# qutech/filter_functions

Measured on AMD Instinct MI355X. Metric: filter-function elements/sec (n_seg*n_omega*n_nops*d^2) at d=4, higher is better.
Workload: dtype f64

## Files before the change

filter_functions_amd/csrc/post.hip:

```cpp
#include <algorithm>

#include <cstdlib>

#include "ffk_internal.h"

namespace ffk {
namespace {

__global__ void reduce_chunks_kernel(const cplx* __restrict__ Ypart, int chunks, size_t slab,
                                     cplx* __restrict__ Bt) {
    const size_t e = static_cast<size_t>(blockIdx.x)*blockDim.x + threadIdx.x;
    if (e >= slab) return;
    cplx acc = Ypart[e];
    for (int c = 1; c < chunks; ++c) {
        const cplx v = Ypart[static_cast<size_t>(c)*slab + e];
        acc.re += v.re;
        acc.im += v.im;
    }
    Bt[e] = acc;
}

__global__ __launch_bounds__(64) void basis_compact_kernel(const cplx* __restrict__ basis, int d,
                                                           int* __restrict__ nnz,
                                                           int* __restrict__ rows,
                                                           cplx* __restrict__ vals) {
    basis_compact_one(basis, d, blockIdx.x, threadIdx.x, nnz, rows, vals);
}

__global__ __launch_bounds__(256) void reduce_compact_kernel(const cplx* __restrict__ Ypart,
                                                             int chunks, size_t slab,
                                                             cplx* __restrict__ Bt, int nred,
                                                             const cplx* __restrict__ basis, int d,
                                                             int* __restrict__ nnz,
                                                             int* __restrict__ rows,
                                                             cplx* __restrict__ vals) {
    if (static_cast<int>(blockIdx.x) >= nred) {
        if (threadIdx.x < 64)
            basis_compact_one(basis, d, static_cast<int>(blockIdx.x) - nred, threadIdx.x, nnz, rows, vals);
        return;
    }
    const size_t e = static_cast<size_t>(blockIdx.x)*blockDim.x + threadIdx.x;
    if (e >= slab) return;
    cplx acc = Ypart[e];
    for (int c = 1; c < chunks; ++c) {
        const cplx v = Ypart[static_cast<size_t>(c)*slab + e];
        acc.re += v.re;
        acc.im += v.im;
    }
    Bt[e] = acc;
}

__device__ __forceinline__ bool basis_is_sparse(const int* __restrict__ nnz, int N, int dd) {
    int part = 0;
    for (int k = threadIdx.x & 63; k < N; k += 64) part += nnz[k];
#pragma unroll
    for (int off = 32; off > 0; off >>= 1) part += __shfl_xor(part, off, 64);
    return part <= 3*dd;
}

template <int KT>
__global__ __launch_bounds__(64) void expand_sparse_kernel(const cplx* __restrict__ Bt,
                                                           const int* __restrict__ nnz,
                                                           const int* __restrict__ rows,
                                                           const cplx* __restrict__ vals, int N,
                                                           int dd, int W, cplx* __restrict__ R,
                                                           int want_sparse) {
    if (want_sparse >= 0 && basis_is_sparse(nnz, N, dd) != (want_sparse != 0)) return;
    const int w = blockIdx.x*64 + threadIdx.x;
    const int a = blockIdx.y;
    if (w >= W) return;
    const cplx* b = Bt + static_cast<size_t>(a)*dd*W + w;
    for (int kk = 0; kk < KT; ++kk) {
        const int k = blockIdx.z*KT + kk;
        if (k >= N) break;
        const int n = nnz[k];
        const int* rk = rows + static_cast<size_t>(k)*dd;
        const cplx* vk = vals + static_cast<size_t>(k)*dd;
        cplx acc0 = {0.0, 0.0}, acc1 = {0.0, 0.0};
        int q = 0;
        for (; q + 1 < n; q += 2) {
            cmac(acc0, vk[q], b[static_cast<size_t>(rk[q])*W]);
            cmac(acc1, vk[q + 1], b[static_cast<size_t>(rk[q + 1])*W]);
        }
        if (q < n) cmac(acc0, vk[q], b[static_cast<size_t>(rk[q])*W]);
        R[(static_cast<size_t>(a)*N + k)*W + w] = {acc0.re + acc1.re, acc0.im + acc1.im};
    }
}
// ... 442 lines not shown

}

hipError_t launch_reduce_chunks(const cplx* Ypart, int chunks, size_t slab, cplx* Bt,
                                hipStream_t stream) {
    const int block = 256;
    hipLaunchKernelGGL(reduce_chunks_kernel, dim3(static_cast<unsigned>((slab + block - 1)/block)),
                       dim3(block), 0, stream, Ypart, chunks, slab, Bt);
    return hipGetLastError();
}

size_t expand_workspace_bytes(int N, int d) {
    const size_t dd = static_cast<size_t>(d)*d;
    return align_up(sizeof(int)*N) + align_up(sizeof(int)*N*dd) + align_up(sizeof(cplx)*N*dd);
}

namespace {
struct CompactWs {
    int* nnz;
    int* rows;
    cplx* vals;
};
CompactWs slice_compact_ws(void* ws, int N, int d) {
    const size_t dd = static_cast<size_t>(d)*d;
    unsigned char* p = static_cast<unsigned char*>(ws);
    CompactWs out;
    out.nnz = reinterpret_cast<int*>(p);
    p += align_up(sizeof(int)*N);
    out.rows = reinterpret_cast<int*>(p);
    p += align_up(sizeof(int)*N*dd);
    out.vals = reinterpret_cast<cplx*>(p);
    return out;
}
}

hipError_t launch_reduce_and_compact(const cplx* Ypart, int chunks, size_t slab, cplx* Bt,
                                     const cplx* basis, int N, int d, void* ws, hipStream_t stream) {
    const CompactWs c = slice_compact_ws(ws, N, d);
    const int block = 256;
    const int nred = static_cast<int>((slab + block - 1)/block);
    hipLaunchKernelGGL(reduce_compact_kernel, dim3(nred + N), dim3(block), 0, stream, Ypart, chunks,
                       slab, Bt, nred, basis, d, c.nnz, c.rows, c.vals);
    return hipGetLastError();
}

void expand_workspace_slices(void* ws, int N, int d, int** nnz, int** rows, cplx** vals) {
    const CompactWs cw = slice_compact_ws(ws, N, d);
    *nnz = cw.nnz;
    *rows = cw.rows;
    *vals = cw.vals;
}

__global__ __launch_bounds__(64) void expand_chunks_kernel(const cplx* __restrict__ Ypart, int chunks,
                                                           size_t slab, const int* __restrict__ nnz,
                                                           const int* __restrict__ rows,
                                                           const cplx* __restrict__ vals, int N,
                                                           int dd, int W, cplx* __restrict__ R) {
    const int w = blockIdx.x*64 + threadIdx.x;
    const int a = blockIdx.y, k = blockIdx.z;
    if (w >= W) return;
    const cplx* b = Ypart + static_cast<size_t>(a)*dd*W + w;
    const int n = nnz[k];
    const int* rk = rows + static_cast<size_t>(k)*dd;
    const cplx* vk = vals + static_cast<size_t>(k)*dd;
    auto summed = [&](int e) {
        cplx acc = b[static_cast<size_t>(e)*W];
        for (int z = 1; z < chunks; ++z) {
            const cplx v = b[z*slab + static_cast<size_t>(e)*W];
            acc.re += v.re;
            acc.im += v.im;
        }
        return acc;
    };
    cplx acc0 = {0.0, 0.0}, acc1 = {0.0, 0.0};
    int q = 0;
    for (; q + 1 < n; q += 2) {
        cmac(acc0, vk[q], summed(rk[q]));
        cmac(acc1, vk[q + 1], summed(rk[q + 1]));
    }
    if (q < n) cmac(acc0, vk[q], summed(rk[q]));
    R[(static_cast<size_t>(a)*N + k)*W + w] = {acc0.re + acc1.re, acc0.im + acc1.im};
}

__device__ __forceinline__ void expand_ff_tile(const cplx* __restrict__ Ypart, int chunks, size_t slab,
                                               const int* __restrict__ nnz, const int* __restrict__ rows,
                                               const cplx* __restrict__ vals, int N, int dd, int W, int A,
                                               int kt, cplx* __restrict__ R, cplx* __restrict__ F) {
    extern __shared__ __attribute__((aligned(16))) unsigned char lds_raw[];
    cplx* rl = reinterpret_cast<cplx*>(lds_raw);
    __builtin_amdgcn_s_setprio(3);
    cplx* ys = rl + static_cast<size_t>(A)*N*16;
    const int wl = threadIdx.x & 15;
    const int kl = (threadIdx.x >> 4) % kt, al = (threadIdx.x >> 4) / kt;
    const int at = (blockDim.x >> 4) / kt;
    const int w = blockIdx.x*16 + wl;
    const int wc = w < W ? w : W - 1;
    for (int idx = threadIdx.x >> 4; idx < A*dd; idx += blockDim.x >> 4) {
        const cplx* b = Ypart + static_cast<size_t>(idx)*W + wc;
        cplx acc = b[0];
        for (int z = 1; z < chunks; ++z) {
            const cplx v = b[z*slab];
            acc.re += v.re;
            acc.im += v.im;
        }
        ys[static_cast<size_t>(idx)*16 + wl] = acc;
    }
    __syncthreads();
    for (int a = al; a < A; a += at) {
        const cplx* ya = ys + static_cast<size_t>(a)*dd*16 + wl;
        for (int k = kl; k < N; k += kt) {
            const int n = nnz[k];
            const int* rk = rows + static_cast<size_t>(k)*dd;
            const cplx* vk = vals + static_cast<size_t>(k)*dd;
            auto summed = [&](int e) { return ya[e*16]; };
            cplx acc0 = {0.0, 0.0}, acc1 = {0.0, 0.0};
            int q = 0;
            for (; q + 1 < n; q += 2) {
                cmac(acc0, vk[q], summed(rk[q]));
                cmac(acc1, vk[q + 1], summed(rk[q + 1]));
            }
            if (q < n) cmac(acc0, vk[q], summed(rk[q]));
            const cplx r = {acc0.re + acc1.re, acc0.im + acc1.im};
            rl[(static_cast<size_t>(a)*N + k)*16 + wl] = r;
            if (w < W) R[(static_cast<size_t>(a)*N + k)*W + w] = r;
        }
    }
    __syncthreads();
    if (w >= W) return;
    const int npairs = A*(A + 1)/2;
    const int lanes = blockDim.x >> 4;
    for (int p = threadIdx.x >> 4; p < npairs; p += lanes) {
        int a = 0, rem = p;
        while (rem >= A - a) {
            rem -= A - a;
            ++a;
        }
        const int b = a + rem;
        const cplx* ra = rl + static_cast<size_t>(a)*N*16 + wl;
        const cplx* rb = rl + static_cast<size_t>(b)*N*16 + wl;
        cplx acc = {0.0, 0.0};
        for (int k = 0; k < N; ++k) cmac_conj(acc, ra[k*16], rb[k*16]);
        if (a == b) acc.im = 0.0;
        F[(static_cast<size_t>(a)*A + b)*W + w] = acc;
        if (a != b) F[(static_cast<size_t>(b)*A + a)*W + w] = {acc.re, -acc.im};
    }
}

__global__ __launch_bounds__(256) void expand_ff_kernel(const cplx* __restrict__ Ypart, int chunks,
                                                         size_t slab, const int* __restrict__ nnz,
                                                         const int* __restrict__ rows,
                                                         const cplx* __restrict__ vals, int N, int dd,
                                                         int W, int A, int kt, cplx* __restrict__ R,
                                                         cplx* __restrict__ F) {
    expand_ff_tile(Ypart, chunks, slab, nnz, rows, vals, N, dd, W, A, kt, R, F);
}

__global__ __launch_bounds__(256) void expand_ff_pulses_kernel(const cplx* __restrict__ Ypart, int chunks,
                                                                size_t slab, const int* __restrict__ nnz,
                                                                const int* __restrict__ rows,
                                                                const cplx* __restrict__ vals, int N, int dd,
                                                                int W, int A, int kt, cplx* __restrict__ R,
                                                                cplx* __restrict__ F) {
    const size_t p = blockIdx.y;
    expand_ff_tile(Ypart + p*chunks*slab, chunks, slab, nnz, rows, vals, N, dd, W, A, kt,
                   R + p*A*N*W, F + p*A*A*W);
}

bool expand_ff_supported(int A, int N) {
    return static_cast<size_t>(A)*2*N*16*sizeof(cplx) <= 128*1024;
}

hipError_t launch_expand_ff(const cplx* Ypart, int chunks, size_t slab, int A, int N, int d, int W,
                            cplx* R, cplx* F, void* ws, hipStream_t stream) {
    if (!expand_ff_supported(A, N)) return hipErrorInvalidValue;
    const CompactWs cw = slice_compact_ws(ws, N, d);
    const int kt = N >= 16 ? 16 : (N >= 8 ? 8 : 4);
    const int at = std::max(1, std::min(A, 16/kt));
    const size_t lds = static_cast<size_t>(A)*(N + d*d)*16*sizeof(cplx);
    if (lds > 160*1024) return hipErrorInvalidValue;
    if (lds > 48*1024) {
        hipError_t err = hipFuncSetAttribute(reinterpret_cast<const void*>(expand_ff_kernel),
                                             hipFuncAttributeMaxDynamicSharedMemorySize,
                                             static_cast<int>(lds));
        if (err != hipSuccess) return err;
    }
    hipLaunchKernelGGL(expand_ff_kernel, dim3((W + 15)/16), dim3(16*kt*at), lds, stream, Ypart,
                       chunks, slab, cw.nnz, cw.rows, cw.vals, N, d*d, W, A, kt, R, F);
    return hipGetLastError();
}

hipError_t launch_expand_ff_pulses(const cplx* Ypart, int chunks, size_t slab, int A, int N, int d, int W,
                                   int P, cplx* R, cplx* F, void* ws, hipStream_t stream) {
    if (!expand_ff_supported(A, N) || P < 1 || P > 65535) return hipErrorInvalidValue;
    const CompactWs cw = slice_compact_ws(ws, N, d);
    const int kt = N >= 16 ? 16 : (N >= 8 ? 8 : 4);
    const int at = std::max(1, std::min(A, 16/kt));
    const size_t lds = static_cast<size_t>(A)*(N + d*d)*16*sizeof(cplx);
    if (lds > 160*1024) return hipErrorInvalidValue;
    if (lds > 48*1024) {
        hipError_t err = hipFuncSetAttribute(reinterpret_cast<const void*>(expand_ff_pulses_kernel),
                                             hipFuncAttributeMaxDynamicSharedMemorySize,
                                             static_cast<int>(lds));
        if (err != hipSuccess) return err;
    }
    hipLaunchKernelGGL(expand_ff_pulses_kernel, dim3((W + 15)/16, P), dim3(16*kt*at), lds, stream, Ypart,
                       chunks, slab, cw.nnz, cw.rows, cw.vals, N, d*d, W, A, kt, R, F);
    return hipGetLastError();
}

__global__ __launch_bounds__(256) void expand_lds_kernel(const cplx* __restrict__ Ypart, int chunks,
                                                         size_t slab, const int* __restrict__ nnz,
                                                         const int* __restrict__ rows,
                                                         const cplx* __restrict__ vals, int N, int dd,
                                                         int W, cplx* __restrict__ R, int want_sparse) {
    extern __shared__ __attribute__((aligned(16))) unsigned char lds_raw[];
    if (want_sparse >= 0 && basis_is_sparse(nnz, N, dd) != (want_sparse != 0)) return;
    cplx* yl = reinterpret_cast<cplx*>(lds_raw);
    const int wl = threadIdx.x & 15, kl = threadIdx.x >> 4;
    const int a = blockIdx.y;
    const int w = blockIdx.x*16 + wl;
    const int wc = w < W ? w : W - 1;
    const cplx* b = Ypart + static_cast<size_t>(a)*dd*W + wc;
    for (int e = kl; e < dd; e += 16) {
        cplx acc = b[static_cast<size_t>(e)*W];
        for (int z = 1; z < chunks; ++z) {
            const cplx v = b[z*slab + static_cast<size_t>(e)*W];
            acc.re += v.re;
            acc.im += v.im;
        }
        yl[e*16 + wl] = acc;
    }
    __syncthreads();
    if (w >= W) return;
    for (int k = kl; k < N; k += 16) {
        const int n = nnz[k];
        const int* rk = rows + static_cast<size_t>(k)*dd;
        const cplx* vk = vals + static_cast<size_t>(k)*dd;
        cplx acc0 = {0.0, 0.0}, acc1 = {0.0, 0.0};
        int q = 0;
        for (; q + 1 < n; q += 2) {
            cmac(acc0, vk[q], yl[rk[q]*16 + wl]);
            cmac(acc1, vk[q + 1], yl[rk[q + 1]*16 + wl]);
        }
        if (q < n) cmac(acc0, vk[q], yl[rk[q]*16 + wl]);
        R[(static_cast<size_t>(a)*N + k)*W + w] = {acc0.re + acc1.re, acc0.im + acc1.im};
    }
}

hipError_t launch_expand_lds(const cplx* Ypart, int chunks, size_t slab, int A, int N, int d, int W,
                             cplx* R, void* ws, hipStream_t stream, int want_sparse = -1) {
    if (A > 65535) return hipErrorInvalidValue;
    const CompactWs cw = slice_compact_ws(ws, N, d);
    const size_t lds = static_cast<size_t>(d)*d*16*sizeof(cplx);
    if (lds > 48*1024) {
        hipError_t err = hipFuncSetAttribute(reinterpret_cast<const void*>(expand_lds_kernel),
                                             hipFuncAttributeMaxDynamicSharedMemorySize,
                                             static_cast<int>(lds));
        if (err != hipSuccess) return err;
    }
    hipLaunchKernelGGL(expand_lds_kernel, dim3((W + 15)/16, A), dim3(256), lds, stream, Ypart, chunks,
                       slab, cw.nnz, cw.rows, cw.vals, N, d*d, W, R, want_sparse);
    return hipGetLastError();
}


hipError_t launch_expand_chunks(const cplx* Ypart, int chunks, size_t slab, int A, int N, int d,
                                int W, cplx* R, void* ws, hipStream_t stream) {
    if (A > 65535 || N > 65535) return hipErrorInvalidValue;
    if (d >= 8 && d <= kMaxD)
        return launch_expand_lds(Ypart, chunks, slab, A, N, d, W, R, ws, stream);
    const CompactWs cw = slice_compact_ws(ws, N, d);
    hipLaunchKernelGGL(expand_chunks_kernel, dim3((W + 63)/64, A, N), dim3(64), 0, stream, Ypart,
                       chunks, slab, cw.nnz, cw.rows, cw.vals, N, d*d, W, R);
    return hipGetLastError();
}

hipError_t launch_expand(const cplx* Bt, const cplx* basis, int A2, int N, int d, int W, cplx* R,
                         void* ws, bool compacted, hipStream_t stream) {
    if (A2 > 65535) return hipErrorInvalidValue;
    const size_t dd = static_cast<size_t>(d)*d;
    const CompactWs cw = slice_compact_ws(ws, N, d);
    int* nnz = cw.nnz;
    int* rows = cw.rows;
    cplx* vals = cw.vals;
    if (!compacted)
        hipLaunchKernelGGL(basis_compact_kernel, dim3(N), dim3(64), 0, stream, basis, d, nnz, rows, vals);
    if (d >= 8 && d <= kMaxD) {
        hipError_t err = launch_expand_lds(Bt, 1, 0, A2, N, d, W, R, ws, stream, 0);
        if (err != hipSuccess) return err;
// ... 125 lines not shown
```

filter_functions_amd/csrc/prep.hip:

```cpp
#include "ffk_internal.h"

namespace ffk {
namespace {

template <int D>
__device__ void prologue_segment(const cplx (*V)[D], cplx (*Q)[D], cplx (*T)[D], cplx (*BV)[D],
                                 int g, int lane, const double* __restrict__ eigvals,
                                 const cplx* __restrict__ n_opers,
                                 const double* __restrict__ n_coeffs,
                                 const double* __restrict__ dt, const double* __restrict__ t, int G,
                                 int A, double* __restrict__ segtab, cplx* __restrict__ Tc,
                                 cplx* __restrict__ ops, cplx* __restrict__ n_opers_transformed,
                                 cplx* __restrict__ eigvecs_propagated, bool with_noise_ops = true,
                                 cplx* __restrict__ wfold = nullptr) {
    constexpr int S = seg_stride(D);
    double* st = segtab + static_cast<size_t>(g)*S;
    if (lane == 0) {
        st[0] = dt[g];
        st[1] = t[g];
    }
    cplx eb = {1.0, 0.0};
    for (int e = lane; e < D*D; e += 64) {
        const double dE = eigvals[static_cast<size_t>(g)*D + e / D] - eigvals[static_cast<size_t>(g)*D + e % D];
        double sb, cb;
        sincos_pi(0.5*(dE*dt[g]), &sb, &cb);
        st[seg_rec(e)] = dE;
        st[seg_rec(e) + 1] = sb;
        st[seg_rec(e) + 2] = cb;
        st[seg_rec(e) + 3] = 0.0;
        eb = {cb, sb};
    }
    if (lane < 2) st[2 + lane] = 0.0;
    for (int e = 4 + 4*D*D + lane; e < S; e += 64) st[e] = 0.0;

    for (int e = lane; e < D*D; e += 64) {
        const int m = e / D, j = e % D;
        cplx acc = {0.0, 0.0};
#pragma unroll
        for (int k = 0; k < D; ++k) cmac_conj(acc, V[k][m], Q[k][j]);
        T[m][j] = acc;
        Tc[static_cast<size_t>(g)*D*D + e] = {acc.re, -acc.im};
        ops[static_cast<size_t>(g)*(1 + A)*D*D + e] = acc;
        if (eigvecs_propagated)
            eigvecs_propagated[static_cast<size_t>(g)*D*D + j*D + m] = {acc.re, -acc.im};
    }
    __syncthreads();

    if (!with_noise_ops) return;
    const bool fold = D == 4 && wfold != nullptr;
    if (fold) {
        if (lane < D*D) Q[lane / D][lane % D] = eb;
        __syncthreads();
    }
    for (int a = 0; a < A; ++a) {
        const cplx* B = n_opers + static_cast<size_t>(a)*D*D;
        const double s = n_coeffs ? n_coeffs[static_cast<size_t>(a)*G + g] : 1.0;
        for (int e = lane; e < D*D; e += 64) {
            const int i = e / D, n = e % D;
            cplx acc = {0.0, 0.0};
#pragma unroll
            for (int k = 0; k < D; ++k) cmac(acc, B[i*D + k], V[k][n]);
            BV[i][n] = acc;
        }
        __syncthreads();
        cplx bbar = {0.0, 0.0};
        for (int e = lane; e < D*D; e += 64) {
            const int m = e / D, n = e % D;
            cplx acc = {0.0, 0.0};
#pragma unroll
            for (int k = 0; k < D; ++k) cmac_conj(acc, V[k][m], BV[k][n]);
            acc.re *= s;
            acc.im *= s;
            ops[(static_cast<size_t>(g)*(1 + A) + 1 + a)*D*D + e] = acc;
            if (n_opers_transformed)
                n_opers_transformed[(static_cast<size_t>(a)*G + g)*D*D + e] = acc;
            if (fold) bbar = acc;
        }
        __syncthreads();
        if (fold) {
            if (lane < D*D) BV[lane / D][lane % D] = bbar;
            __syncthreads();
            if constexpr (D == 4) {
                const int m = lane >> 4, n = (lane >> 2) & 3, j = lane & 3;
                const cplx et = cmul(Q[m][n], T[n][j]);
                const cplx w = cmul(BV[m][n], et);
                wfold[(static_cast<size_t>(g)*A + a)*64 + n*16 + m*4 + j] = w;
            }
            __syncthreads();
        }
    }
}

template <int D>
__global__ __launch_bounds__(64) void prologue_kernel(
    const double* __restrict__ eigvals, const cplx* __restrict__ eigvecs,
    const cplx* __restrict__ propagators, const cplx* __restrict__ n_opers,
    const double* __restrict__ n_coeffs, const double* __restrict__ dt,
    const double* __restrict__ t, int G, int A, double* __restrict__ segtab,
    cplx* __restrict__ Tc, cplx* __restrict__ ops, cplx* __restrict__ n_opers_transformed,
    cplx* __restrict__ eigvecs_propagated, bool with_noise_ops, cplx* __restrict__ wfold) {
    __shared__ cplx V[D][D];
    __shared__ cplx Q[D][D];
    __shared__ cplx T[D][D];
    __shared__ cplx BV[D][D];
    const int g = blockIdx.x;
    const int lane = threadIdx.x;
    for (int e = lane; e < D*D; e += 64) {
        V[e / D][e % D] = eigvecs[static_cast<size_t>(g)*D*D + e];
        Q[e / D][e % D] = propagators[static_cast<size_t>(g)*D*D + e];
    }
    __syncthreads();
    prologue_segment<D>(V, Q, T, BV, g, lane, eigvals, n_opers, n_coeffs, dt, t, G, A, segtab, Tc,
                        ops, n_opers_transformed, eigvecs_propagated, with_noise_ops, wfold);
}

template <int D>
__global__ __launch_bounds__(64) void noise_ops_kernel(const cplx* __restrict__ eigvecs,
                                                       const cplx* __restrict__ n_opers,
                                                       const double* __restrict__ n_coeffs, int G,
                                                       int A, cplx* __restrict__ ops,
                                                       cplx* __restrict__ n_opers_transformed) {
    __shared__ cplx V[D][D];
    __shared__ cplx BV[D][D];
    __builtin_amdgcn_s_setprio(3);
    const int g = blockIdx.x, a = blockIdx.y, lane = threadIdx.x;
    for (int e = lane; e < D*D; e += 64) V[e / D][e % D] = eigvecs[static_cast<size_t>(g)*D*D + e];
    __syncthreads();
    const cplx* B = n_opers + static_cast<size_t>(a)*D*D;
    const double s = n_coeffs ? n_coeffs[static_cast<size_t>(a)*G + g] : 1.0;
    for (int e = lane; e < D*D; e += 64) {
        const int i = e / D, n = e % D;
        cplx acc = {0.0, 0.0};
#pragma unroll
        for (int k = 0; k < D; ++k) cmac(acc, B[i*D + k], V[k][n]);
        BV[i][n] = acc;
    }
    __syncthreads();
    for (int e = lane; e < D*D; e += 64) {
        const int m = e / D, n = e % D;
        cplx acc = {0.0, 0.0};
#pragma unroll
        for (int k = 0; k < D; ++k) cmac_conj(acc, V[k][m], BV[k][n]);
        acc.re *= s;
        acc.im *= s;
        ops[(static_cast<size_t>(g)*(1 + A) + 1 + a)*D*D + e] = acc;
        if (n_opers_transformed)
            n_opers_transformed[(static_cast<size_t>(a)*G + g)*D*D + e] = acc;
    }
}

constexpr int kNoiseOpsKernelMinD = 12;
inline bool split_noise_ops(int d, int A) { return d >= kNoiseOpsKernelMinD && A >= 2 && A <= 65535; }

template <int D>
__device__ __forceinline__ void apply_prologue_segment(
    const cplx* __restrict__ Qloc, const cplx* __restrict__ totals, int G, int L,
    cplx* __restrict__ Qout, const double* __restrict__ eigvals, const cplx* __restrict__ eigvecs,
    const cplx* __restrict__ n_opers, const double* __restrict__ n_coeffs,
    const double* __restrict__ dt, const double* __restrict__ t, int A,
    double* __restrict__ segtab, cplx* __restrict__ Tc, cplx* __restrict__ ops,
    bool with_noise_ops, cplx* __restrict__ wfold, const int g) {
    __builtin_amdgcn_s_setprio(3);
    __shared__ cplx E[2][D][D];
    __shared__ cplx M[D][D];
    __shared__ cplx V[D][D];
    __shared__ cplx Q[D][D];
    __shared__ cplx T[D][D];
    __shared__ cplx BV[D][D];
    constexpr int kBatch = 16;
    constexpr bool kTree = D <= 8;
    extern __shared__ __attribute__((aligned(16))) unsigned char tot_raw[];
    cplx (*tot)[D][D] = reinterpret_cast<cplx (*)[D][D]>(tot_raw);
    const int lane = threadIdx.x;
    const int c = g / L;
    for (int e = lane; e < D*D; e += 64) E[0][e / D][e % D] = {(e / D == e % D) ? 1.0 : 0.0, 0.0};
    int b = 0;
    if constexpr (kTree) {
        constexpr int DD = D*D, PER = 64/DD;
        for (int e = lane; e < c*DD; e += 64) (&tot[0][0][0])[e] = totals[e];
        __syncthreads();
        int n = c;
        while (n > 1) {
            const int pairs = n >> 1;
            for (int j0 = 0; j0 < pairs; j0 += PER) {
                const int jj = j0 + lane/DD, e = lane % DD, i = e / D, k = e % D;
                const bool act = lane < PER*DD && jj < pairs;
                cplx acc = {0.0, 0.0};
                if (act) {
#pragma unroll
                    for (int x = 0; x < D; ++x) cmac(acc, tot[2*jj + 1][i][x], tot[2*jj][x][k]);
                }
                __syncthreads();
                if (act) tot[jj][i][k] = acc;
                __syncthreads();
            }
            if (n & 1) {
                const cplx* from = &tot[n - 1][0][0] + (lane < DD ? lane : 0);
                const double carry_re = from->re, carry_im = from->im;
                __syncthreads();
                if (lane < DD) (&tot[pairs][0][0])[lane] = {carry_re, carry_im};
                __syncthreads();
            }
            n = pairs + (n & 1);
        }
        if (c > 0) {
            for (int e = lane; e < DD; e += 64) E[0][e / D][e % D] = tot[0][e / D][e % D];
            __syncthreads();
        }
    } else {
    for (int kb = 0; kb < c; kb += kBatch) {
        const int nb = min(kBatch, c - kb);
        __syncthreads();
        for (int e = lane; e < nb*D*D; e += 64)
            (&tot[0][0][0])[e] = totals[static_cast<size_t>(kb)*D*D + e];
        __syncthreads();
        for (int k = 0; k < nb; ++k) {
            for (int e = lane; e < D*D; e += 64) {
                const int i = e / D, j = e % D;
                cplx acc = {0.0, 0.0};
#pragma unroll
                for (int x = 0; x < D; ++x) cmac(acc, tot[k][i][x], E[b][x][j]);
                E[b ^ 1][i][j] = acc;
            }
            __syncthreads();
            b ^= 1;
        }
    }
    }
    for (int e = lane; e < D*D; e += 64) M[e / D][e % D] = Qloc[static_cast<size_t>(g + 1)*D*D + e];
    if (g == 0)
        for (int e = lane; e < D*D; e += 64) Qout[e] = {(e / D == e % D) ? 1.0 : 0.0, 0.0};
    __syncthreads();
    for (int e = lane; e < D*D; e += 64) {
        const int i = e / D, j = e % D;
        cplx acc = {0.0, 0.0};
#pragma unroll
        for (int x = 0; x < D; ++x) cmac(acc, M[i][x], E[b][x][j]);
        Qout[static_cast<size_t>(g + 1)*D*D + e] = acc;
    }
    if (segtab == nullptr) return;
    __syncthreads();
    if (g % L == 0) {
        for (int e = lane; e < D*D; e += 64) Q[e / D][e % D] = E[b][e / D][e % D];
    } else {
        for (int e = lane; e < D*D; e += 64) M[e / D][e % D] = Qloc[static_cast<size_t>(g)*D*D + e];
        __syncthreads();
        for (int e = lane; e < D*D; e += 64) {
            const int i = e / D, j = e % D;
            cplx acc = {0.0, 0.0};
#pragma unroll
            for (int x = 0; x < D; ++x) cmac(acc, M[i][x], E[b][x][j]);
            Q[i][j] = acc;
        }
    }
    for (int e = lane; e < D*D; e += 64) V[e / D][e % D] = eigvecs[static_cast<size_t>(g)*D*D + e];
    __syncthreads();
    prologue_segment<D>(V, Q, T, BV, g, lane, eigvals, n_opers, n_coeffs, dt, t, G, A, segtab, Tc,
                        ops, nullptr, nullptr, with_noise_ops, wfold);
}

template <int D>
__global__ __launch_bounds__(64) void apply_prologue_kernel(
    const cplx* __restrict__ Qloc, const cplx* __restrict__ totals, int G, int L,
    cplx* __restrict__ Qout, const double* __restrict__ eigvals, const cplx* __restrict__ eigvecs,
    const cplx* __restrict__ n_opers, const double* __restrict__ n_coeffs,
    const double* __restrict__ dt, const double* __restrict__ t, int A,
    double* __restrict__ segtab, cplx* __restrict__ Tc, cplx* __restrict__ ops,
    const cplx* __restrict__ basis, int* __restrict__ nnz, int* __restrict__ rows,
    cplx* __restrict__ vals, bool with_noise_ops, cplx* __restrict__ wfold) {
    if (static_cast<int>(blockIdx.x) >= G) {
        basis_compact_one(basis, D, static_cast<int>(blockIdx.x) - G, threadIdx.x, nnz, rows, vals);
        return;
    }
    apply_prologue_segment<D>(Qloc, totals, G, L, Qout, eigvals, eigvecs, n_opers, n_coeffs, dt, t, A, segtab, Tc,
                              ops, with_noise_ops, wfold, blockIdx.x);
}

template <int D>
__global__ __launch_bounds__(64) void apply_prologue_pulses_kernel(
    const cplx* __restrict__ Qloc, const cplx* __restrict__ totals, int G, int L, int nchunks,
    cplx* __restrict__ Qout, const double* __restrict__ eigvals, const cplx* __restrict__ eigvecs,
    const cplx* __restrict__ n_opers, const double* __restrict__ n_coeffs,
    const double* __restrict__ dt, const double* __restrict__ t, int A,
    double* __restrict__ segtab, cplx* __restrict__ Tc, cplx* __restrict__ ops,
    const cplx* __restrict__ basis, int* __restrict__ nnz, int* __restrict__ rows,
    cplx* __restrict__ vals, cplx* __restrict__ wfold) {
    const size_t p = blockIdx.y;
    if (static_cast<int>(blockIdx.x) >= G) {
        if (p == 0) basis_compact_one(basis, D, static_cast<int>(blockIdx.x) - G, threadIdx.x, nnz, rows, vals);
        return;
    }
    constexpr size_t DD = D*D;
    apply_prologue_segment<D>(Qloc + p*(G + 1)*DD, totals + p*nchunks*DD, G, L, Qout + p*(G + 1)*DD,
                              eigvals + p*G*D, eigvecs + p*G*DD, n_opers + p*A*DD, n_coeffs + p*A*G, dt + p*G,
                              t + p*(G + 1), A, segtab + p*G*seg_stride(D), Tc + p*G*DD, ops + p*G*(1 + A)*DD,
                              true, wfold ? wfold + p*G*A*64 : nullptr, blockIdx.x);
}

template <int D>
__global__ __launch_bounds__(64) void basis_transformed_kernel(const cplx* __restrict__ Tc,
                                                               const cplx* __restrict__ basis,
                                                               int N, cplx* __restrict__ out) {
    __shared__ cplx T[D][D];
    __shared__ cplx C[D][D];
    __shared__ cplx TC[D][D];
    const int g = blockIdx.x, k = blockIdx.y, lane = threadIdx.x;
    for (int e = lane; e < D*D; e += 64) {
        const cplx v = Tc[static_cast<size_t>(g)*D*D + e];
        T[e / D][e % D] = {v.re, -v.im};
        C[e / D][e % D] = basis[static_cast<size_t>(k)*D*D + e];
    }
    __syncthreads();
    for (int e = lane; e < D*D; e += 64) {
        const int i = e / D, j = e % D;
        cplx acc = {0.0, 0.0};
#pragma unroll
        for (int a = 0; a < D; ++a) cmac(acc, T[i][a], C[a][j]);
        TC[i][j] = acc;
    }
    __syncthreads();
    for (int e = lane; e < D*D; e += 64) {
        const int i = e / D, j = e % D;
        cplx acc = {0.0, 0.0};
#pragma unroll
        for (int a = 0; a < D; ++a) {
            const cplx tj = T[j][a];
            cmac_conj(acc, tj, TC[i][a]);
        }
        out[(static_cast<size_t>(g)*N + k)*D*D + e] = acc;
    }
}

__global__ void phase_integral_kernel(const double* __restrict__ omega, int W,
                                      const double* __restrict__ segtab, int d, int S,
                                      cplx* __restrict__ phase_factors,
                                      cplx* __restrict__ integral) {
    const int g = blockIdx.x;
    const int w = blockIdx.y*blockDim.x + threadIdx.x;
    if (w >= W) return;
    const double* st = segtab + static_cast<size_t>(g)*S;
    const double om = omega[w];
    if (phase_factors) phase_factors[static_cast<size_t>(g)*W + w] = cexp(om*st[1]);
    if (integral) {
        cplx* out = integral + (static_cast<size_t>(g)*W + w)*d*d;
        for (int e = 0; e < d*d; ++e) out[e] = first_order_integral(om, st[seg_rec(e)], st[0]);
    }
}

}

__global__ __launch_bounds__(64) void fold_w8_kernel(const double* __restrict__ segtab, const cplx* __restrict__ ops,
                                                     int A, cplx* __restrict__ wfold) {
    constexpr int D = 8, DD = 64, S = seg_stride(8);
    const int g = blockIdx.x, a = blockIdx.y, lane = threadIdx.x;
    const cplx* src = ops + static_cast<size_t>(g)*(1 + A)*DD;
    const double* r = segtab + static_cast<size_t>(g)*S + seg_rec(lane);
    const cplx x = src[static_cast<size_t>(1 + a)*DD + lane];
    const double sb = r[1], cb = r[2];
    const int m = lane >> 3, n = lane & 7;
    const int base = ((m >> 2)*2 + (n >> 2))*2*64 + 4*(n & 3) + 16*(m & 3);
    const cplx bt = cmul(x, cplx{cb, sb});
    cplx* out = wfold + (static_cast<size_t>(g)*A + a)*512;
#pragma unroll
    for (int i = 0; i < D; ++i) {
        const cplx t = src[m*D + i];
        out[base + (i >> 2)*64 + (i & 3)] = cmul(bt, cplx{t.re, -t.im});
    }
}

hipError_t launch_fold_w8(const double* segtab, const cplx* ops, int G, int A, cplx* wfold, hipStream_t stream) {
    hipLaunchKernelGGL(fold_w8_kernel, dim3(G, A), dim3(64), 0, stream, segtab, ops, A, wfold);
    return hipGetLastError();
}

hipError_t launch_prologue(const double* eigvals, const cplx* eigvecs, const cplx* propagators,
                           const cplx* n_opers, const double* n_coeffs, const double* dt,
                           const double* t, int G, int d, int A, double* segtab, cplx* Tc,
                           cplx* ops, cplx* n_opers_transformed, cplx* eigvecs_propagated,
                           hipStream_t stream, cplx* wfold) {
    if (generic_dimension(d))
        return launch_prologue_generic(eigvals, eigvecs, propagators, n_opers, n_coeffs, dt, t, G, d, A, segtab,
                                       Tc, ops, n_opers_transformed, eigvecs_propagated, stream);
    switch (d) {
#define FFK_CASE(D)                                                                             \
    case D:                                                                                     \
        hipLaunchKernelGGL(prologue_kernel<D>, dim3(G), dim3(64), 0, stream, eigvals, eigvecs,  \
                           propagators, n_opers, n_coeffs, dt, t, G, A, segtab, Tc, ops,        \
                           n_opers_transformed, eigvecs_propagated, !split_noise_ops(D, A),     \
                           D == 4 ? wfold : nullptr);                                           \
        if (split_noise_ops(D, A))                                                              \
            hipLaunchKernelGGL(noise_ops_kernel<D>, dim3(G, A), dim3(64), 0, stream, eigvecs,   \
                               n_opers, n_coeffs, G, A, ops, n_opers_transformed);              \
        break;
        FFK_CASE(2) FFK_CASE(3) FFK_CASE(4) FFK_CASE(5) FFK_CASE(6) FFK_CASE(7) FFK_CASE(8)
        FFK_CASE(9) FFK_CASE(10) FFK_CASE(11) FFK_CASE(12) FFK_CASE(13) FFK_CASE(14)
        FFK_CASE(15) FFK_CASE(16)
#undef FFK_CASE
        default:
            return hipErrorInvalidValue;
    }
    if (d == 8 && wfold != nullptr) return launch_fold_w8(segtab, ops, G, A, wfold, stream);
    return hipGetLastError();
}

hipError_t launch_apply_prologue_compact(const cplx* Qloc, const cplx* totals, int G, int d, cplx* Q,
                                         const double* eigvals, const cplx* eigvecs,
                                         const cplx* n_opers, const double* n_coeffs,
                                         const double* dt, const double* t, int A, double* segtab,
                                         cplx* Tc, cplx* ops, const cplx* basis, int N, void* ews,
                                         hipStream_t stream, cplx* wfold) {
    const int L = front_chunk(d);
    int* nnz = nullptr;
    int* rows = nullptr;
    cplx* vals = nullptr;
    int extra = 0;
    if (basis) {
        expand_workspace_slices(ews, N, d, &nnz, &rows, &vals);
        extra = N;
    }
    switch (d) {
#define FFK_CASE(D)                                                                              \
    case D:                                                                                      \
        if (D > 8) {    \
            hipError_t e = hipFuncSetAttribute(reinterpret_cast<const void*>(apply_prologue_kernel<D>), \
                                               hipFuncAttributeMaxDynamicSharedMemorySize,       \
                                               static_cast<int>(sizeof(cplx)*D*D*16));           \
            if (e != hipSuccess) return e;                                                       \
        }                                                                                        \
        hipLaunchKernelGGL(apply_prologue_kernel<D>, dim3(G + extra), dim3(64),                  \
                           sizeof(cplx)*D*D*(D <= 8 ? (G + L - 1)/L : 16), stream, Qloc,         \
                           totals, G, L, Q, eigvals, eigvecs, n_opers, n_coeffs, dt, t, A,       \
                           segtab, Tc, ops, basis, nnz, rows, vals, !split_noise_ops(D, A),      \
                           D == 4 ? wfold : nullptr);                                            \
        if (split_noise_ops(D, A))                                                               \
            hipLaunchKernelGGL(noise_ops_kernel<D>, dim3(G, A), dim3(64), 0, stream, eigvecs,    \
                               n_opers, n_coeffs, G, A, ops, nullptr);                           \
        break;
        FFK_CASE(2) FFK_CASE(3) FFK_CASE(4) FFK_CASE(5) FFK_CASE(6) FFK_CASE(7) FFK_CASE(8)
        FFK_CASE(9) FFK_CASE(10) FFK_CASE(11) FFK_CASE(12) FFK_CASE(13) FFK_CASE(14)
        FFK_CASE(15) FFK_CASE(16)
#undef FFK_CASE
        default:
            return hipErrorInvalidValue;
    }
    if (d == 8 && wfold != nullptr) return launch_fold_w8(segtab, ops, G, A, wfold, stream);
    return hipGetLastError();
}

hipError_t launch_apply_prologue_compact_pulses(const cplx* Qloc, const cplx* totals, int G, int P, int d,
                                                cplx* Q, const double* eigvals, const cplx* eigvecs,
                                                const cplx* n_opers, const double* n_coeffs, const double* dt,
                                                const double* t, int A, double* segtab, cplx* Tc, cplx* ops,
                                                const cplx* basis, int N, void* ews, hipStream_t stream,
                                                cplx* wfold) {
    const int L = front_chunk(d);
    const int nchunks = (G + L - 1)/L;
    if (P < 1 || P > 65535 || !basis) return hipErrorInvalidValue;
    int* nnz = nullptr;
    int* rows = nullptr;
    cplx* vals = nullptr;
    expand_workspace_slices(ews, N, d, &nnz, &rows, &vals);
    switch (d) {
#define FFK_CASE(D)                                                                              \
    case D:                                                                                      \
        if (D > 8) {                                                                             \
            hipError_t e = hipFuncSetAttribute(reinterpret_cast<const void*>(apply_prologue_pulses_kernel<D>), \
                                               hipFuncAttributeMaxDynamicSharedMemorySize,       \
                                               static_cast<int>(sizeof(cplx)*D*D*16));           \
            if (e != hipSuccess) return e;                                                       \
        }                                                                                        \
        hipLaunchKernelGGL(apply_prologue_pulses_kernel<D>, dim3(G + N, P), dim3(64),            \
                           sizeof(cplx)*D*D*(D <= 8 ? nchunks : 16), stream, Qloc, totals, G, L, \
                           nchunks, Q, eigvals, eigvecs, n_opers, n_coeffs, dt, t, A, segtab, Tc, \
                           ops, basis, nnz, rows, vals, D == 4 ? wfold : nullptr);               \
        break;
        FFK_CASE(2) FFK_CASE(3) FFK_CASE(4) FFK_CASE(5) FFK_CASE(6) FFK_CASE(7) FFK_CASE(8)
        FFK_CASE(9) FFK_CASE(10) FFK_CASE(11) FFK_CASE(12) FFK_CASE(13) FFK_CASE(14)
        FFK_CASE(15) FFK_CASE(16)
#undef FFK_CASE
        default:
            return hipErrorInvalidValue;
    }
    if (d == 8 && wfold != nullptr) return launch_fold_w8(segtab, ops, P*G, A, wfold, stream);
    return hipGetLastError();
}

hipError_t launch_apply_prologue(const cplx* Qloc, const cplx* totals, int G, int d, cplx* Q,
                                 const double* eigvals, const cplx* eigvecs, const cplx* n_opers,
                                 const double* n_coeffs, const double* dt, const double* t, int A,
                                 double* segtab, cplx* Tc, cplx* ops, hipStream_t stream) {
    return launch_apply_prologue_compact(Qloc, totals, G, d, Q, eigvals, eigvecs, n_opers, n_coeffs,
                                         dt, t, A, segtab, Tc, ops, nullptr, 0, nullptr, stream);
}

hipError_t launch_basis_transformed(const cplx* Tc, const cplx* basis, int G, int N, int d,
                                    cplx* out, hipStream_t stream) {
    if (N > 65535) return hipErrorInvalidValue;
    switch (d) {
#define FFK_CASE(D)                                                                            \
    case D:                                                                                    \
        hipLaunchKernelGGL(basis_transformed_kernel<D>, dim3(G, N), dim3(64), 0, stream, Tc,   \
                           basis, N, out);                                                     \
        break;
        FFK_CASE(2) FFK_CASE(3) FFK_CASE(4) FFK_CASE(5) FFK_CASE(6) FFK_CASE(7) FFK_CASE(8)
        FFK_CASE(9) FFK_CASE(10) FFK_CASE(11) FFK_CASE(12) FFK_CASE(13) FFK_CASE(14)
        FFK_CASE(15) FFK_CASE(16)
#undef FFK_CASE
        default:
            return hipErrorInvalidValue;
    }
    return hipGetLastError();
}

hipError_t launch_phase_and_integral(const double* omega, int W, const double* segtab, int G,
                                     int d, cplx* phase_factors, cplx* integral,
                                     hipStream_t stream) {
    if (!phase_factors && !integral) return hipSuccess;
    const int block = 128;
    if ((W + block - 1)/block > 65535) return hipErrorInvalidValue;
    hipLaunchKernelGGL(phase_integral_kernel, dim3(G, (W + block - 1)/block), dim3(block), 0,
                       stream, omega, W, segtab, d, seg_stride(d), phase_factors, integral);
    return hipGetLastError();
}

}
```

Before: 928.5 billion.

## Stage sparse lists in LDS, unroll partial sums, and hoist prologue global loads

The expand kernel now copies the compact basis lists (vals, rows, nnz) into shared memory with async LDS DMA when they fit. It also sums the chunk partials with templated, unrolled loads so several loads are in flight at once, and unrolls the conjugate dot loop. In the prologue kernel, global loads of totals, Qloc, eigvecs, eigvals, dt/t and the first noise operators are issued up front into registers and parked in extra LDS, which drops several sync points. The aim is to hide global memory latency at the cost of more LDS use, more registers and more complex code.

```diff
diff --git a/filter_functions_amd/csrc/post.hip b/filter_functions_amd/csrc/post.hip
--- a/filter_functions_amd/csrc/post.hip
+++ b/filter_functions_amd/csrc/post.hip
@@ -3,6 +3,7 @@
 #include <cstdlib>
 
 #include "ffk_internal.h"
+#include "ffk_mfma_util.h"
 
 namespace ffk {
 namespace {
@@ -611,49 +612,115 @@
     R[(static_cast<size_t>(a)*N + k)*W + w] = {acc0.re + acc1.re, acc0.im + acc1.im};
 }
 
+template <int CH, int IB>
+__device__ __forceinline__ void sum_partials(const cplx* __restrict__ b0, int chunks, size_t slab, int W, int count,
+                                             int first, int step, int wl, cplx* __restrict__ ys) {
+    if constexpr (CH > 0) {
+        for (int i0 = first; i0 < count; i0 += IB*step) {
+            double vr[IB][CH], vi[IB][CH];
+#pragma unroll
+            for (int i = 0; i < IB; ++i) {
+                const cplx* b = b0 + static_cast<size_t>(min(i0 + i*step, count - 1))*W;
+#pragma unroll
+                for (int z = 0; z < CH; ++z) {
+                    vr[i][z] = b[z*slab].re;
+                    vi[i][z] = b[z*slab].im;
+                }
+            }
+#pragma unroll
+            for (int i = 0; i < IB; ++i) {
+                cplx acc = {vr[i][0], vi[i][0]};
+#pragma unroll
+                for (int z = 1; z < CH; ++z) {
+                    acc.re += vr[i][z];
+                    acc.im += vi[i][z];
+                }
+                ys[static_cast<size_t>(min(i0 + i*step, count - 1))*16 + wl] = acc;
+            }
+        }
+    } else {
+        for (int idx = first; idx < count; idx += step) {
+            const cplx* b = b0 + static_cast<size_t>(idx)*W;
+            cplx acc = {0.0, 0.0};
+            for (int z0 = 0; z0 < chunks; z0 += 4) {
+                double vr[4], vi[4];
+#pragma unroll
+                for (int z = 0; z < 4; ++z) {
+                    const cplx* from = b + min(z0 + z, chunks - 1)*slab;
+                    vr[z] = from->re;
+                    vi[z] = from->im;
+                }
+#pragma unroll
+                for (int z = 0; z < 4; ++z) {
+                    if (z0 + z == 0) {
+                        acc = {vr[0], vi[0]};
+                    } else if (z0 + z < chunks) {
+                        acc.re += vr[z];
+                        acc.im += vi[z];
+                    }
+                }
+            }
+            ys[static_cast<size_t>(idx)*16 + wl] = acc;
+        }
+    }
+}
+
 __device__ __forceinline__ void expand_ff_tile(const cplx* __restrict__ Ypart, int chunks, size_t slab,
                                                const int* __restrict__ nnz, const int* __restrict__ rows,
                                                const cplx* __restrict__ vals, int N, int dd, int W, int A,
-                                               int kt, cplx* __restrict__ R, cplx* __restrict__ F) {
+                                               int kt, cplx* __restrict__ R, cplx* __restrict__ F, int stage_lists) {
     extern __shared__ __attribute__((aligned(16))) unsigned char lds_raw[];
     cplx* rl = reinterpret_cast<cplx*>(lds_raw);
     __builtin_amdgcn_s_setprio(3);
     cplx* ys = rl + static_cast<size_t>(A)*N*16;
+    cplx* vals_l = ys + static_cast<size_t>(A)*dd*16;
+    int* rows_l = reinterpret_cast<int*>(vals_l + static_cast<size_t>(N)*dd);
+    int* nnz_l = rows_l + ((N*dd + 3) & ~3);
     const int wl = threadIdx.x & 15;
     const int kl = (threadIdx.x >> 4) % kt, al = (threadIdx.x >> 4) / kt;
     const int at = (blockDim.x >> 4) / kt;
     const int w = blockIdx.x*16 + wl;
     const int wc = w < W ? w : W - 1;
-    for (int idx = threadIdx.x >> 4; idx < A*dd; idx += blockDim.x >> 4) {
-        const cplx* b = Ypart + static_cast<size_t>(idx)*W + wc;
-        cplx acc = b[0];
-        for (int z = 1; z < chunks; ++z) {
-            const cplx v = b[z*slab];
-            acc.re += v.re;
-            acc.im += v.im;
-        }
-        ys[static_cast<size_t>(idx)*16 + wl] = acc;
-    }
+    if (stage_lists) {
+        const int tid = threadIdx.x, wave = tid >> 6;
+        if (tid < N*dd) lds_dma16(vals + tid, vals_l + wave*64);
+        if (4*tid < N*dd) lds_dma16(rows + 4*tid, rows_l + wave*256);
+        if (4*tid < N) lds_dma16(nnz + 4*tid, nnz_l + wave*256);
+    }
+    const cplx* b0 = Ypart + wc;
+    const int first = threadIdx.x >> 4, step = blockDim.x >> 4;
+    switch (chunks) {
+        case 1: sum_partials<1, 4>(b0, chunks, slab, W, A*dd, first, step, wl, ys); break;
+        case 2: sum_partials<2, 4>(b0, chunks, slab, W, A*dd, first, step, wl, ys); break;
+        case 3: sum_partials<3, 2>(b0, chunks, slab, W, A*dd, first, step, wl, ys); break;
+        case 4: sum_partials<4, 2>(b0, chunks, slab, W, A*dd, first, step, wl, ys); break;
+        default: sum_partials<0, 1>(b0, chunks, slab, W, A*dd, first, step, wl, ys); break;
+    }
+    lds_dma_wait();
     __syncthreads();
-    for (int a = al; a < A; a += at) {
-        const cplx* ya = ys + static_cast<size_t>(a)*dd*16 + wl;
-        for (int k = kl; k < N; k += kt) {
-            const int n = nnz[k];
-            const int* rk = rows + static_cast<size_t>(k)*dd;
-            const cplx* vk = vals + static_cast<size_t>(k)*dd;
-            auto summed = [&](int e) { return ya[e*16]; };
-            cplx acc0 = {0.0, 0.0}, acc1 = {0.0, 0.0};
-            int q = 0;
-            for (; q + 1 < n; q += 2) {
-                cmac(acc0, vk[q], summed(rk[q]));
-                cmac(acc1, vk[q + 1], summed(rk[q + 1]));
+    auto expand = [&](const int* nz, const int* rw, const cplx* vl) {
+        for (int a = al; a < A; a += at) {
+            const cplx* ya = ys + static_cast<size_t>(a)*dd*16 + wl;
+            for (int k = kl; k < N; k += kt) {
+                const int n = nz[k];
+                const int* rk = rw + static_cast<size_t>(k)*dd;
+                const cplx* vk = vl + static_cast<size_t>(k)*dd;
+                auto summed = [&](int e) { return ya[e*16]; };
+                cplx acc0 = {0.0, 0.0}, acc1 = {0.0, 0.0};
+                int q = 0;
+                for (; q + 1 < n; q += 2) {
+                    cmac(acc0, vk[q], summed(rk[q]));
+                    cmac(acc1, vk[q + 1], summed(rk[q + 1]));
+                }
+                if (q < n) cmac(acc0, vk[q], summed(rk[q]));
+                const cplx r = {acc0.re + acc1.re, acc0.im + acc1.im};
+                rl[(static_cast<size_t>(a)*N + k)*16 + wl] = r;
+                if (w < W) R[(static_cast<size_t>(a)*N + k)*W + w] = r;
             }
-            if (q < n) cmac(acc0, vk[q], summed(rk[q]));
-            const cplx r = {acc0.re + acc1.re, acc0.im + acc1.im};
-            rl[(static_cast<size_t>(a)*N + k)*16 + wl] = r;
-            if (w < W) R[(static_cast<size_t>(a)*N + k)*W + w] = r;
-        }
-    }
+        }
+    };
+    if (stage_lists) expand(nnz_l, rows_l, vals_l);
+    else expand(nnz, rows, vals);
     __syncthreads();
     if (w >= W) return;
     const int npairs = A*(A + 1)/2;
@@ -668,6 +735,7 @@
         const cplx* ra = rl + static_cast<size_t>(a)*N*16 + wl;
         const cplx* rb = rl + static_cast<size_t>(b)*N*16 + wl;
         cplx acc = {0.0, 0.0};
+#pragma unroll 4
         for (int k = 0; k < N; ++k) cmac_conj(acc, ra[k*16], rb[k*16]);
         if (a == b) acc.im = 0.0;
         F[(static_cast<size_t>(a)*A + b)*W + w] = acc;
@@ -680,8 +748,8 @@
                                                          const int* __restrict__ rows,
                                                          const cplx* __restrict__ vals, int N, int dd,
                                                          int W, int A, int kt, cplx* __restrict__ R,
-                                                         cplx* __restrict__ F) {
-    expand_ff_tile(Ypart, chunks, slab, nnz, rows, vals, N, dd, W, A, kt, R, F);
+                                                         cplx* __restrict__ F, int stage_lists) {
+    expand_ff_tile(Ypart, chunks, slab, nnz, rows, vals, N, dd, W, A, kt, R, F, stage_lists);
 }
 
 __global__ __launch_bounds__(256) void expand_ff_pulses_kernel(const cplx* __restrict__ Ypart, int chunks,
@@ -689,10 +757,17 @@
                                                                 const int* __restrict__ rows,
                                                                 const cplx* __restrict__ vals, int N, int dd,
                                                                 int W, int A, int kt, cplx* __restrict__ R,
-                                                                cplx* __restrict__ F) {
+                                                                cplx* __restrict__ F, int stage_lists) {
     const size_t p = blockIdx.y;
     expand_ff_tile(Ypart + p*chunks*slab, chunks, slab, nnz, rows, vals, N, dd, W, A, kt,
-                   R + p*A*N*W, F + p*A*A*W);
+                   R + p*A*N*W, F + p*A*A*W, stage_lists);
+}
+
+static size_t expand_ff_list_bytes(size_t tiles, int N, int d, int threads) {
+    const size_t entries = static_cast<size_t>(N)*d*d;
+    const size_t bytes = entries*sizeof(cplx) + align_up(entries*sizeof(int), 16) + align_up(sizeof(int)*N, 16);
+    if (entries > static_cast<size_t>(threads) || tiles + bytes > 56*1024) return 0;
+    return bytes;
 }
 
 bool expand_ff_supported(int A, int N) {
@@ -705,7 +780,9 @@
     const CompactWs cw = slice_compact_ws(ws, N, d);
     const int kt = N >= 16 ? 16 : (N >= 8 ? 8 : 4);
     const int at = std::max(1, std::min(A, 16/kt));
-    const size_t lds = static_cast<size_t>(A)*(N + d*d)*16*sizeof(cplx);
+    const size_t tiles = static_cast<size_t>(A)*(N + d*d)*16*sizeof(cplx);
+    const size_t lists = expand_ff_list_bytes(tiles, N, d, 16*kt*at);
+    const size_t lds = tiles + lists;
     if (lds > 160*1024) return hipErrorInvalidValue;
     if (lds > 48*1024) {
         hipError_t err = hipFuncSetAttribute(reinterpret_cast<const void*>(expand_ff_kernel),
@@ -714,7 +791,7 @@
         if (err != hipSuccess) return err;
     }
     hipLaunchKernelGGL(expand_ff_kernel, dim3((W + 15)/16), dim3(16*kt*at), lds, stream, Ypart,
-                       chunks, slab, cw.nnz, cw.rows, cw.vals, N, d*d, W, A, kt, R, F);
+                       chunks, slab, cw.nnz, cw.rows, cw.vals, N, d*d, W, A, kt, R, F, lists ? 1 : 0);
     return hipGetLastError();
 }
 
@@ -724,7 +801,9 @@
     const CompactWs cw = slice_compact_ws(ws, N, d);
     const int kt = N >= 16 ? 16 : (N >= 8 ? 8 : 4);
     const int at = std::max(1, std::min(A, 16/kt));
-    const size_t lds = static_cast<size_t>(A)*(N + d*d)*16*sizeof(cplx);
+    const size_t tiles = static_cast<size_t>(A)*(N + d*d)*16*sizeof(cplx);
+    const size_t lists = expand_ff_list_bytes(tiles, N, d, 16*kt*at);
+    const size_t lds = tiles + lists;
     if (lds > 160*1024) return hipErrorInvalidValue;
     if (lds > 48*1024) {
         hipError_t err = hipFuncSetAttribute(reinterpret_cast<const void*>(expand_ff_pulses_kernel),
@@ -733,7 +812,7 @@
         if (err != hipSuccess) return err;
     }
     hipLaunchKernelGGL(expand_ff_pulses_kernel, dim3((W + 15)/16, P), dim3(16*kt*at), lds, stream, Ypart,
-                       chunks, slab, cw.nnz, cw.rows, cw.vals, N, d*d, W, A, kt, R, F);
+                       chunks, slab, cw.nnz, cw.rows, cw.vals, N, d*d, W, A, kt, R, F, lists ? 1 : 0);
     return hipGetLastError();
 }
 
diff --git a/filter_functions_amd/csrc/prep.hip b/filter_functions_amd/csrc/prep.hip
--- a/filter_functions_amd/csrc/prep.hip
+++ b/filter_functions_amd/csrc/prep.hip
@@ -3,27 +3,28 @@
 namespace ffk {
 namespace {
 
-template <int D>
-__device__ void prologue_segment(const cplx (*V)[D], cplx (*Q)[D], cplx (*T)[D], cplx (*BV)[D],
-                                 int g, int lane, const double* __restrict__ eigvals,
-                                 const cplx* __restrict__ n_opers,
-                                 const double* __restrict__ n_coeffs,
-                                 const double* __restrict__ dt, const double* __restrict__ t, int G,
-                                 int A, double* __restrict__ segtab, cplx* __restrict__ Tc,
-                                 cplx* __restrict__ ops, cplx* __restrict__ n_opers_transformed,
-                                 cplx* __restrict__ eigvecs_propagated, bool with_noise_ops = true,
-                                 cplx* __restrict__ wfold = nullptr) {
+constexpr int kHoistOps = 3;
+
+template <int D, bool PRE = false>
+__device__ __forceinline__ void prologue_segment(
+    const cplx (*V)[D], cplx (*Q)[D], cplx (*T)[D], cplx (*BV)[D], int g, int lane,
+    const double* __restrict__ eigvals, const cplx* __restrict__ n_opers, const double* __restrict__ n_coeffs,
+    const double* __restrict__ dt, const double* __restrict__ t, int G, int A, double* __restrict__ segtab,
+    cplx* __restrict__ Tc, cplx* __restrict__ ops, cplx* __restrict__ n_opers_transformed,
+    cplx* __restrict__ eigvecs_propagated, bool with_noise_ops, cplx* __restrict__ wfold, const cplx* Bs,
+    const double dE_pre, const double dtg, const double tg, const double (&b_s)[kHoistOps]) {
     constexpr int S = seg_stride(D);
     double* st = segtab + static_cast<size_t>(g)*S;
     if (lane == 0) {
-        st[0] = dt[g];
-        st[1] = t[g];
+        st[0] = PRE ? dtg : dt[g];
+        st[1] = PRE ? tg : t[g];
     }
     cplx eb = {1.0, 0.0};
     for (int e = lane; e < D*D; e += 64) {
-        const double dE = eigvals[static_cast<size_t>(g)*D + e / D] - eigvals[static_cast<size_t>(g)*D + e % D];
+        const double dE = PRE ? dE_pre
+                              : eigvals[static_cast<size_t>(g)*D + e / D] - eigvals[static_cast<size_t>(g)*D + e % D];
         double sb, cb;
-        sincos_pi(0.5*(dE*dt[g]), &sb, &cb);
+        sincos_pi(0.5*(dE*(PRE ? dtg : dt[g])), &sb, &cb);
         st[seg_rec(e)] = dE;
         st[seg_rec(e) + 1] = sb;
         st[seg_rec(e) + 2] = cb;
@@ -54,12 +55,25 @@
     }
     for (int a = 0; a < A; ++a) {
         const cplx* B = n_opers + static_cast<size_t>(a)*D*D;
-        const double s = n_coeffs ? n_coeffs[static_cast<size_t>(a)*G + g] : 1.0;
+        const bool staged = PRE && a < kHoistOps;
+        double s = 1.0;
+        if (staged) {
+#pragma unroll
+            for (int x = 0; x < kHoistOps; ++x) s = a == x ? b_s[x] : s;
+            s = n_coeffs ? s : 1.0;
+        } else {
+            s = n_coeffs ? n_coeffs[static_cast<size_t>(a)*G + g] : 1.0;
+        }
         for (int e = lane; e < D*D; e += 64) {
             const int i = e / D, n = e % D;
             cplx acc = {0.0, 0.0};
-#pragma unroll
-            for (int k = 0; k < D; ++k) cmac(acc, B[i*D + k], V[k][n]);
+            if (staged) {
+#pragma unroll
+                for (int k = 0; k < D; ++k) cmac(acc, Bs[(a*D + i)*D + k], V[k][n]);
+            } else {
+#pragma unroll
+                for (int k = 0; k < D; ++k) cmac(acc, B[i*D + k], V[k][n]);
+            }
             BV[i][n] = acc;
         }
         __syncthreads();
@@ -110,8 +124,10 @@
         Q[e / D][e % D] = propagators[static_cast<size_t>(g)*D*D + e];
     }
     __syncthreads();
+    const double none[kHoistOps] = {};
     prologue_segment<D>(V, Q, T, BV, g, lane, eigvals, n_opers, n_coeffs, dt, t, G, A, segtab, Tc,
-                        ops, n_opers_transformed, eigvecs_propagated, with_noise_ops, wfold);
+                        ops, n_opers_transformed, eigvecs_propagated, with_noise_ops, wfold, nullptr, 0.0, 0.0, 0.0,
+                        none);
 }
 
 template <int D>
@@ -173,18 +189,89 @@
     cplx (*tot)[D][D] = reinterpret_cast<cplx (*)[D][D]>(tot_raw);
     const int lane = threadIdx.x;
     const int c = g / L;
+    constexpr int DD = D*D, PER = (DD + 63)/64;
+    const bool full = segtab != nullptr;
+    cplx* Bpark = &tot[(G + L - 1)/L][0][0];
+    constexpr int kTotFirst = 4;
+    double tr[kTotFirst], ti[kTotFirst];
+    if constexpr (kTree) {
+        const cplx* tsrc = c > 0 ? totals : Qloc;
+        const int last = c > 0 ? c*DD - 1 : 0;
+#pragma unroll
+        for (int r = 0; r < kTotFirst; ++r) {
+            const unsigned off = static_cast<unsigned>(min(lane + 64*r, last))*static_cast<unsigned>(sizeof(cplx));
+            const cplx* from = reinterpret_cast<const cplx*>(reinterpret_cast<const char*>(tsrc) + off);
+            tr[r] = from->re;
+            ti[r] = from->im;
+        }
+    }
+    double qn_re[PER], qn_im[PER], qg_re[PER], qg_im[PER], v_re[PER], v_im[PER];
+    const cplx* vsrc = full ? eigvecs + static_cast<size_t>(g)*DD : Qloc;
+#pragma unroll
+    for (int r = 0; r < PER; ++r) {
+        const int ec = min(lane + 64*r, DD - 1);
+        const cplx* qn = Qloc + static_cast<size_t>(g + 1)*DD + ec;
+        const cplx* qg = Qloc + static_cast<size_t>(g)*DD + ec;
+        qn_re[r] = qn->re;
+        qn_im[r] = qn->im;
+        qg_re[r] = qg->re;
+        qg_im[r] = qg->im;
+        v_re[r] = vsrc[ec].re;
+        v_im[r] = vsrc[ec].im;
+    }
+    double ev_m = 0.0, ev_n = 0.0, dtg = 0.0, tg = 0.0;
+    double b_re[kHoistOps], b_im[kHoistOps], b_s[kHoistOps];
+    if constexpr (kTree) {
+        const int ec = min(lane, DD - 1);
+        const double* spare = reinterpret_cast<const double*>(Qloc);
+        const double* evsrc = full ? eigvals + static_cast<size_t>(g)*D : spare;
+        ev_m = evsrc[ec / D];
+        ev_n = evsrc[ec % D];
+        dtg = *(full ? dt + g : spare);
+        tg = *(full ? t + g : spare);
+        const bool opers = full && with_noise_ops && A > 0;
+#pragma unroll
+        for (int a = 0; a < kHoistOps; ++a) {
+            const int ac = min(a, A - 1);
+            const cplx* bp = (opers ? n_opers + static_cast<size_t>(ac)*DD : Qloc) + ec;
+            b_re[a] = bp->re;
+            b_im[a] = bp->im;
+            b_s[a] = *(opers && n_coeffs ? n_coeffs + static_cast<size_t>(ac)*G + g : spare);
+        }
+    } else {
+#pragma unroll
+        for (int a = 0; a < kHoistOps; ++a) b_re[a] = b_im[a] = b_s[a] = 0.0;
+    }
     for (int e = lane; e < D*D; e += 64) E[0][e / D][e % D] = {(e / D == e % D) ? 1.0 : 0.0, 0.0};
+    if constexpr (kTree) {
+#pragma unroll
+        for (int r = 0; r < kTotFirst; ++r) (&tot[0][0][0])[min(lane + 64*r, c > 0 ? c*DD - 1 : 0)] = {tr[r], ti[r]};
+    }
+#pragma unroll
+    for (int r = 0; r < PER; ++r) {
+        const int e = lane + 64*r;
+        if (e < DD) {
+            M[e / D][e % D] = {qn_re[r], qn_im[r]};
+            BV[e / D][e % D] = {qg_re[r], qg_im[r]};
+            V[e / D][e % D] = {v_re[r], v_im[r]};
+            if constexpr (kTree) {
+#pragma unroll
+                for (int a = 0; a < kHoistOps; ++a) Bpark[a*DD + e] = {b_re[a], b_im[a]};
+            }
+        }
+    }
+    const double dE = ev_m - ev_n;
     int b = 0;
     if constexpr (kTree) {
-        constexpr int DD = D*D, PER = 64/DD;
-        for (int e = lane; e < c*DD; e += 64) (&tot[0][0][0])[e] = totals[e];
+        constexpr int PAIRS = 64/DD;
+        for (int e = lane + 64*kTotFirst; e < c*DD; e += 64) (&tot[0][0][0])[e] = totals[e];
         __syncthreads();
         int n = c;
         while (n > 1) {
             const int pairs = n >> 1;
-            for (int j0 = 0; j0 < pairs; j0 += PER) {
+            for (int j0 = 0; j0 < pairs; j0 += PAIRS) {
                 const int jj = j0 + lane/DD, e = lane % DD, i = e / D, k = e % D;
-                const bool act = lane < PER*DD && jj < pairs;
+                const bool act = lane < PAIRS*DD && jj < pairs;
                 cplx acc = {0.0, 0.0};
                 if (act) {
 #pragma unroll
@@ -227,7 +314,6 @@
         }
     }
     }
-    for (int e = lane; e < D*D; e += 64) M[e / D][e % D] = Qloc[static_cast<size_t>(g + 1)*D*D + e];
     if (g == 0)
         for (int e = lane; e < D*D; e += 64) Qout[e] = {(e / D == e % D) ? 1.0 : 0.0, 0.0};
     __syncthreads();
@@ -239,24 +325,20 @@
         Qout[static_cast<size_t>(g + 1)*D*D + e] = acc;
     }
     if (segtab == nullptr) return;
-    __syncthreads();
     if (g % L == 0) {
         for (int e = lane; e < D*D; e += 64) Q[e / D][e % D] = E[b][e / D][e % D];
     } else {
-        for (int e = lane; e < D*D; e += 64) M[e / D][e % D] = Qloc[static_cast<size_t>(g)*D*D + e];
-        __syncthreads();
         for (int e = lane; e < D*D; e += 64) {
             const int i = e / D, j = e % D;
             cplx acc = {0.0, 0.0};
 #pragma unroll
-            for (int x = 0; x < D; ++x) cmac(acc, M[i][x], E[b][x][j]);
+            for (int x = 0; x < D; ++x) cmac(acc, BV[i][x], E[b][x][j]);
             Q[i][j] = acc;
         }
     }
-    for (int e = lane; e < D*D; e += 64) V[e / D][e % D] = eigvecs[static_cast<size_t>(g)*D*D + e];
-    __syncthreads();
-    prologue_segment<D>(V, Q, T, BV, g, lane, eigvals, n_opers, n_coeffs, dt, t, G, A, segtab, Tc,
-                        ops, nullptr, nullptr, with_noise_ops, wfold);
+    __syncthreads();
+    prologue_segment<D, kTree>(V, Q, T, BV, g, lane, eigvals, n_opers, n_coeffs, dt, t, G, A, segtab, Tc, ops, nullptr,
+                               nullptr, with_noise_ops, wfold, Bpark, dE, dtg, tg, b_s);
 }
 
 template <int D>
@@ -403,6 +485,10 @@
     return hipGetLastError();
 }
 
+static size_t prologue_dynamic_lds(int D, int nchunks) {
+    return sizeof(cplx)*D*D*(D <= 8 ? nchunks + kHoistOps : 16);
+}
+
 hipError_t launch_apply_prologue_compact(const cplx* Qloc, const cplx* totals, int G, int d, cplx* Q,
                                          const double* eigvals, const cplx* eigvecs,
                                          const cplx* n_opers, const double* n_coeffs,
@@ -421,14 +507,15 @@
     switch (d) {
 #define FFK_CASE(D)                                                                              \
     case D:                                                                                      \
-        if (D > 8) {    \
+                  \
+        if (D > 8 || prologue_dynamic_lds(D, (G + L - 1)/L) > 48*1024) {                         \
             hipError_t e = hipFuncSetAttribute(reinterpret_cast<const void*>(apply_prologue_kernel<D>), \
                                                hipFuncAttributeMaxDynamicSharedMemorySize,       \
-                                               static_cast<int>(sizeof(cplx)*D*D*16));           \
+                                               static_cast<int>(prologue_dynamic_lds(D, (G + L - 1)/L)));  \
             if (e != hipSuccess) return e;                                                       \
         }                                                                                        \
         hipLaunchKernelGGL(apply_prologue_kernel<D>, dim3(G + extra), dim3(64),                  \
-                           sizeof(cplx)*D*D*(D <= 8 ? (G + L - 1)/L : 16), stream, Qloc,         \
+                           prologue_dynamic_lds(D, (G + L - 1)/L), stream, Qloc,                \
                            totals, G, L, Q, eigvals, eigvecs, n_opers, n_coeffs, dt, t, A,       \
                            segtab, Tc, ops, basis, nnz, rows, vals, !split_noise_ops(D, A),      \
                            D == 4 ? wfold : nullptr);                                            \
@@ -463,14 +550,14 @@
     switch (d) {
 #define FFK_CASE(D)                                                                              \
     case D:                                                                                      \
-        if (D > 8) {                                                                             \
+        if (D > 8 || prologue_dynamic_lds(D, nchunks) > 48*1024) {                               \
             hipError_t e = hipFuncSetAttribute(reinterpret_cast<const void*>(apply_prologue_pulses_kernel<D>), \
                                                hipFuncAttributeMaxDynamicSharedMemorySize,       \
-                                               static_cast<int>(sizeof(cplx)*D*D*16));           \
+                                               static_cast<int>(prologue_dynamic_lds(D, nchunks)));  \
             if (e != hipSuccess) return e;                                                       \
         }                                                                                        \
         hipLaunchKernelGGL(apply_prologue_pulses_kernel<D>, dim3(G + N, P), dim3(64),            \
-                           sizeof(cplx)*D*D*(D <= 8 ? nchunks : 16), stream, Qloc, totals, G, L, \
+                           prologue_dynamic_lds(D, nchunks), stream, Qloc, totals, G, L,        \
                            nchunks, Q, eigvals, eigvecs, n_opers, n_coeffs, dt, t, A, segtab, Tc, \
                            ops, basis, nnz, rows, vals, D == 4 ? wfold : nullptr);               \
         break;
```

New measurement: 932.5 billion, median of 6. About the same (+0.4%).
